# Sageblatt/plate_inverse_problem

Hardware: AMD Instinct MI355X
Metric: freq-solves/sec (forward+adjoint) @20k DOF (higher is better)
Workload: dtype f64; 1 GPU; C3: orthotropic CFRP-like plate, sh_i strip 100x20x2 mm + AP1030, 19353 DOF, 4096 freqs in 40-600 Hz (in total, 4096 on rank 0), forward+adjoint, loss MSE_LOG_AFC + gradient; n_dofs=19353, freqs_total=4096, freqs_rank0=4096, chunk=2048, lanes=2, factorisation=symmetric: A = L U, U = diag(U) L^T implicit, Dirichlet nodes decoupled, nnz_lu=589025

## Files before the change

### include/pfr.h

```cpp
#ifndef PFR_H
#define PFR_H

#include <stddef.h>
#include <stdint.h>

#ifdef __cplusplus
extern "C" {
#endif

#define PFR_API __attribute__((visibility("default")))

#define PFR_OK 0
#define PFR_ERR_ARG 1
#define PFR_ERR_SYMBOLIC 2
#define PFR_ERR_HIP 3
#define PFR_ERR_NOMEM 4
#define PFR_ERR_STATE 5

#define PFR_FLAG_BAD_PIVOT 1
#define PFR_FLAG_BACKWARD_ERROR 2
#define PFR_FLAG_BACKWARD_ERROR_ADJ 4

#define PFR_CHECK_FORWARD 1
#define PFR_CHECK_ADJOINT 2
// ... 76 lines not shown

#define PFR_SCHED_FACTOR_COLS 13
#define PFR_SCHED_PAIR_COLS 9
#define PFR_SCHED_CHAIN_COLS 11
#define PFR_SCHED_SOLVE_COLS 5
#define PFR_SCHED_COLS (PFR_SCHED_FACTOR_COLS + PFR_SCHED_PAIR_COLS + PFR_SCHED_CHAIN_COLS + 3 * PFR_SCHED_SOLVE_COLS)
PFR_API int pfr_symbolic_schedule(const pfr_symbolic* sym, int32_t max_batch, int32_t* dst, int64_t capacity_bytes);
PFR_API int pfr_solver_schedule(const pfr_solver* s, int32_t* dst, int64_t capacity_bytes);

PFR_API int pfr_set_prune(pfr_solver* s, int32_t on);
PFR_API int pfr_symbolic_prune(const pfr_symbolic* sym, int32_t max_batch, const double* rhs, int32_t n_support,
                               const int32_t* index, int32_t* mask, int32_t* sched_active, int32_t* sched_rest,
                               int32_t* sched_full, int64_t capacity_bytes);
PFR_API int32_t pfr_solver_active(const pfr_solver* s, int32_t* mask, int64_t capacity);
PFR_API int pfr_solver_schedule_active(const pfr_solver* s, int32_t* dst, int64_t capacity_bytes);

PFR_API int pfr_solve(pfr_solver* s, int32_t batch, const double* data_dev, int64_t data_stride,
                      const double* b_dev, int64_t b_stride, double* x_dev, int32_t transpose,
                      int32_t* flags_dev, void* stream);

PFR_API int pfr_solve_multi(pfr_solver* s, int32_t batch, int32_t nrhs, const double* data_dev,
                            int64_t data_stride, const double* b_dev, int64_t b_stride, int64_t b_rhs_stride,
                            double* x_dev, int64_t x_rhs_stride, int32_t transpose, int32_t* flags_dev,
                            void* stream);
PFR_API int pfr_matvec(pfr_solver* s, int32_t batch, const double* data_dev, int64_t data_stride,
                       const double* x_dev, int64_t x_stride, double* y_dev, int32_t transpose, void* stream);


PFR_API int pfr_set_stiffness(pfr_solver* s, int32_t n_stiff, const double* stiff_dev ,
                              const double* rhs_weights );
// ... 55 lines not shown
```

### plate_inverse_problem_amd/_native.py

```python
from __future__ import annotations

import ctypes as C
import os
import re

import numpy as np

LIB_PATH = os.environ.get("PFR_LIB") or os.path.join(os.path.dirname(os.path.abspath(__file__)), "_lib", "libpfr.so")
HEADER_PATH = os.path.join(os.path.dirname(os.path.dirname(os.path.abspath(__file__))), "include", "pfr.h")

PFR_OK = 0
PFR_FLAG_BAD_PIVOT = 1
PFR_FLAG_BACKWARD_ERROR = 2
PFR_FLAG_BACKWARD_ERROR_ADJ = 4
PFR_CHECK_FORWARD, PFR_CHECK_ADJOINT, PFR_CHECK_REFINE, PFR_CHECK_CORRECT = 1, 2, 4, 8
PFR_CHECK_REFINE_ADJ = 16
LOSS_NONE, LOSS_MSE, LOSS_RMSE, LOSS_MSE_AFC, LOSS_MSE_LOG_AFC, LOSS_COTANGENT = -1, 0, 1, 2, 3, 4
LOSS_IDS = {"MSE": LOSS_MSE, "RMSE": LOSS_RMSE, "MSE_AFC": LOSS_MSE_AFC, "MSE_LOG_AFC": LOSS_MSE_LOG_AFC}
LOSS_CMSE, LOSS_CRMSE, LOSS_CLOG, LOSS_CCOTANGENT = 16, 17, 18, 19
COMPLEX_LOSS_IDS = {"MSE_COMPLEX": LOSS_CMSE, "RMSE_COMPLEX": LOSS_CRMSE, "MSE_LOG_COMPLEX": LOSS_CLOG}

EXPORT = dict(PERM=0, IPERM=1, FRONTS=2, IDX=3, RELPOS=4, ASM_PTR=5, ASM_COL=6, ASM_NZ=7, EA_PTR=8,
              EA_SRC=9, LEVEL_PTR=10, LEVEL_FRONTS=11, DIRICHLET=12, COUPLING=13)

# ... 39 lines not shown
    "pfr_symbolic_options_default": (None, [C.POINTER(SymbolicOptions)]),
    "pfr_symbolic_create": (C.c_int, [C.c_int32, C.c_int64, _I32P, _I32P, C.POINTER(SymbolicOptions), C.POINTER(_P)]),
    "pfr_symbolic_stats_get": (C.c_int, [_P, C.POINTER(SymbolicStats)]),
    "pfr_symbolic_export": (C.c_int, [_P, C.c_int32, _P, C.c_int64]),
    "pfr_symbolic_destroy": (None, [_P]),
    "pfr_solver_create": (C.c_int, [_P, _I32P, _I32P, C.c_int32, C.c_int32, C.POINTER(_P)]),
    "pfr_solver_destroy": (None, [_P]),
    "pfr_solver_workspace_bytes": (C.c_int64, [_P, C.c_int32]),
    "pfr_solver_max_batch": (C.c_int32, [_P]),
    "pfr_symbolic_schedule": (C.c_int, [_P, C.c_int32, _I32P, C.c_int64]),
    "pfr_solver_schedule": (C.c_int, [_P, _I32P, C.c_int64]),
    "pfr_set_prune": (C.c_int, [_P, C.c_int32]),
    "pfr_symbolic_prune": (C.c_int, [_P, C.c_int32, _DP, C.c_int32, _I32P, _I32P, _I32P, _I32P, _I32P, C.c_int64]),
    "pfr_solver_active": (C.c_int32, [_P, _I32P, C.c_int64]),
    "pfr_solver_schedule_active": (C.c_int, [_P, _I32P, C.c_int64]),
    "pfr_solve": (C.c_int, [_P, C.c_int32, _P, C.c_int64, _P, C.c_int64, _P, C.c_int32, _P, _P]),
    "pfr_matvec": (C.c_int, [_P, C.c_int32, _P, C.c_int64, _P, C.c_int64, _P, C.c_int32, _P]),
    "pfr_set_stiffness": (C.c_int, [_P, C.c_int32, _P, _DP]),
    "pfr_combine": (C.c_int, [_P, _DP, _P, _P]),
    "pfr_set_operator": (C.c_int, [_P, _P, _P]),
    "pfr_set_rhs": (C.c_int, [_P, _DP, C.c_double, C.c_double, C.c_double]),
    "pfr_set_functional": (C.c_int, [_P, C.c_int32, _I32P, _DP, C.c_double]),
    "pfr_sweep": (C.c_int, [_P, C.c_int32, _P, C.c_int32, _P, C.c_double, _P, _P, _P, _P, _P]),
    "pfr_sweep_graph_launches": (C.c_int64, [_P]),
    "pfr_stream_order": (C.c_int, [_P, _P]),
    "pfr_sweep_fresh": (C.c_int, [_P, C.c_int32, _P, C.c_int32, _P, C.c_double, _P, _P, _P, _P, _P]),
    "pfr_jacobian_sweep": (C.c_int, [_P, C.c_int32, _P, _P, _P, _P, _P]),
    "pfr_sweep_complex": (C.c_int, [_P, C.c_int32, _P, _DP, C.c_int32, _P, C.c_double, _P, _P, _P, _P, C.c_int32, _P]),
    "pfr_jacobian_sweep_complex": (C.c_int, [_P, C.c_int32, _P, _DP, _P, _P, _P, _P]),
    "pfr_combine_batch": (C.c_int, [_P, C.c_int32, _DP, _P, _P]),
# ... 162 lines not shown
        st = self.stats()
        r, rp = _f64(rhs)
        sup, sp = _i32(np.asarray(support, dtype=np.int32))
        mask = np.zeros(st["n_fronts"], dtype=np.int32)
        cols = sum(len(c) for _, c in SCHEDULE)
        flat = np.zeros((3, st["n_levels"] * cols), dtype=np.int32)
        check(lib().pfr_symbolic_prune(self._h, int(max_batch), rp, int(sup.size), sp, mask.ctypes.data_as(_I32P),
                                       flat[0].ctypes.data_as(_I32P), flat[1].ctypes.data_as(_I32P),
                                       flat[2].ctypes.data_as(_I32P), flat[0].nbytes),
              "pfr_symbolic_prune")

        def table(row):
            return _schedule(st["n_levels"], lambda dst, cap: C.memmove(dst, row.ctypes.data, row.nbytes))
        return mask, table(flat[0]), table(flat[1]), table(flat[2])

    def __del__(self):
        h = getattr(self, "_h", None)
        if h is not None and _lib is not None:
            _lib.pfr_symbolic_destroy(h)
            self._h = None


class Solver:

    def __init__(self, sym: Symbolic, device_index: int, max_batch: int):
        L = lib()
        self.sym = sym
        self.device_index = int(device_index)
        h = _P()
        _, cp = _i32(sym.colptr)
# ... 10 lines not shown
            _lib.pfr_solver_destroy(h)
            self._h = None

    def schedule(self) -> dict:
        return _schedule(self.sym.stats()["n_levels"], lambda dst, cap: check(
            lib().pfr_solver_schedule(self._h, dst, cap), "pfr_solver_schedule"))

    def set_prune(self, on: bool = True):
        check(lib().pfr_set_prune(self._h, int(bool(on))), "pfr_set_prune")

    def active_fronts(self) -> np.ndarray:
        mask = np.zeros(self.sym.stats()["n_fronts"], dtype=np.int32)
        lib().pfr_solver_active(self._h, mask.ctypes.data_as(_I32P), mask.size)
        return mask

    def schedule_active(self) -> dict:
        return _schedule(self.sym.stats()["n_levels"], lambda dst, cap: check(
            lib().pfr_solver_schedule_active(self._h, dst, cap), "pfr_solver_schedule_active"))

    @staticmethod
    def _stream(t):
        import torch
        return torch.cuda.current_stream(t.device).cuda_stream

    def set_stiffness(self, stiff_nz_k, rhs_weights):
        self._keep["stiff"] = stiff_nz_k
        w, wp = _f64(rhs_weights)
        check(lib().pfr_set_stiffness(self._h, int(stiff_nz_k.shape[1]), _ptr(stiff_nz_k), wp), "pfr_set_stiffness")

    def combine(self, coef: np.ndarray, out):
# ... 121 lines not shown
```

### plate_inverse_problem_amd/csrc/api.cpp

```cpp
#include <hip/hip_runtime.h>

#include <algorithm>
#include <array>
#include <cmath>
#include <cstring>
#include <string>
#include <vector>

#include "launch.hpp"

using pfr::DevPattern;
using pfr::Front;
using pfr::Symbolic;
using pfr::Walk;

struct pfr_symbolic {
  Symbolic S;
};

namespace {
thread_local std::string g_last_error;

int fail(int code, const std::string& msg) {
  g_last_error = msg;
// ... 22 lines not shown
  HIP_TRY(hipMalloc(dst, src.size() * sizeof(T)));
  HIP_TRY(hipMemcpy(*dst, src.data(), src.size() * sizeof(T), hipMemcpyHostToDevice));
  return PFR_OK;
}

int64_t round64(int64_t x) { return (x + 63) / 64 * 64; }

}

struct SolverView {
  std::vector<char> active;
  std::vector<int32_t> level_ptr;
  std::vector<int32_t> tile_ptr, blk_ptr, asm_ptr, item_ptr;
  std::vector<void*> mine;
  int32_t* d_walk = nullptr;
  int post_n = 0;
  int2* post_dir = nullptr;
  int32_t* post_dptr = nullptr;
  int2* post_de = nullptr;
  int32_t* d_level_fronts = nullptr;
  int4* d_tiles = nullptr;
  int4* d_items = nullptr;
  int2* d_orec = nullptr;
  int32_t *d_f0_front = nullptr, *d_f0_ptr = nullptr, *d_f0_nz = nullptr;
  int32_t* d_oxp = nullptr;
  int2* d_ox = nullptr;
  int32_t* d_g1 = nullptr;
  int32_t* d_gxp = nullptr;
  int2* d_gx = nullptr;
  int4* d_blocks = nullptr;
// ... 49 lines not shown
  int2* d_de = nullptr;
  int32_t* d_cslot = nullptr;
  double2* Bc = nullptr;
  std::vector<int32_t> front_of_col, front_parent, front_ns, front_f;
  int fn_dot = 1;
  std::vector<int32_t> front_off, front_col0;
  std::vector<double> a_perm;
  double* d_aP = nullptr;
  int32_t* d_noslot = nullptr;
  double2* WVk = nullptr;
  double2* YVk = nullptr;
  double2* fn_parts = nullptr;
  double2* fcoef = nullptr;
  int contract_walk = 1;
  double2* kpart = nullptr;
  double2 *F = nullptr, *WV = nullptr, *X = nullptr, *Y = nullptr, *XA = nullptr, *G = nullptr, *Y2 = nullptr;
  double2* XR = nullptr;
  int32_t *d_rptr = nullptr, *d_ridx = nullptr, *d_rnz = nullptr;
  int32_t *d_cptr = nullptr, *d_cidx = nullptr, *d_cnz = nullptr;
  double2 *DX = nullptr, *DL = nullptr, *Kdir = nullptr;
  int4* d_uent = nullptr;
  int n_uent = 0;
  double* d_se = nullptr;
  int n_kdir = 0;
  double2 *partial = nullptr, *tq = nullptr;
  double *freqs = nullptr, *loss_terms = nullptr;
  double* fr0 = nullptr;
  double2* h0 = nullptr;
  double2 *mscale = nullptr, *cpart = nullptr;
  int scale_corr = 1;
// ... 373 lines not shown
int set_reach(pfr_solver* s, SolverView& v, int which, const std::vector<int32_t>& prows) {
  std::vector<int32_t> mark, list;
  pfr::reach_lists(s->front_of_col, s->front_parent, v.level_ptr, v.level_fronts_host, prows, mark, list,
                   v.reach_ptr[which]);
  v.reach_host[which].assign(mark.begin(), mark.end());
  v.fn_ready = false;
  if (&v == s && s->act) s->act->fn_ready = false;
  pfr::schedule_reach(v.sched, v.reach_ptr, &v != s ? &s->reach_ptr : nullptr);
  HIP_TRY(hipMemcpy(v.d_reach[which], mark.data(), mark.size() * 4, hipMemcpyHostToDevice));
  if (!list.empty()) HIP_TRY(hipMemcpy(v.d_reach_fronts[which], list.data(), list.size() * 4, hipMemcpyHostToDevice));
  return PFR_OK;
}

void run_walk(pfr_solver* s, const SolverView& v, const pfr::ChunkOp& op, const Walk& w, int nvalid, hipStream_t st) {
  const bool fwd = w.sys == Walk::FORWARD;
  const pfr::ResidArgs d{.ptr = fwd ? s->d_rptr : s->d_cptr, .idx = fwd ? s->d_ridx : s->d_cidx,
                         .nzs = fwd ? s->d_rnz : s->d_cnz, .n = s->n, .K = op.K, .M = op.M, .freqs = op.freqs,
                         .data = w.data, .data_stride = w.ds, .nvalid = nvalid, .rhsP = w.rd.rhsP,
                         .beta_re = w.rd.beta_re, .beta_im = w.rd.beta_im, .mass_sum = w.rd.mass_sum, .B = w.rd.B,
                         .b_stride = w.rd.b_stride, .perm = s->P.perm, .G = w.rd.G, .walk = v.d_walk,
                         .se = w.contract ? s->stiff : nullptr, .kpart = w.contract ? s->kpart : nullptr,
                         .glist = w.glist};
  const int n_stiff = w.contract ? s->n_stiff : 0;
  pfr::launch_residual(w.mat, w.rhs, d, n_stiff, s->res_unroll, op.pop, w.X, s->Fc, w.R, w.check ? s->d_berr_acc : nullptr,
                       st, w.Mu, w.Mu ? s->cpart : nullptr);
  if (!w.check) return;
  pfr::launch_berr_finish(s->d_berr_acc, s->Fc, nvalid, s->check_tol,
                          fwd ? PFR_FLAG_BACKWARD_ERROR : PFR_FLAG_BACKWARD_ERROR_ADJ, s->flags,
                          w.q0 >= 0 ? s->berr_out : nullptr, w.q0, w.sys, st);
}

void contract_rows(pfr_solver* s, const double2* lam, const double2* x, int nv, hipStream_t st) {
  pfr::launch_contract_eg(s->d_uent, s->n_uent, s->d_se, s->n_stiff, lam, x, s->Fc, nv, s->partial, st);
}

int upload_view(pfr_solver* s, SolverView& v, const Symbolic& S, const pfr::Plan& pl, const pfr::Knobs& knobs) {
  int rc;
  const size_t own0 = s->owned.size();
  const int nf = (int)S.fronts.size();
  v.active = pl.active;
// ... 29 lines not shown
  if (&v != s) v.mine.assign(s->owned.begin() + own0, s->owned.end());
  return PFR_OK;
}

void release_view(pfr_solver* s, SolverView*& v) {
  if (!v) return;
  (void)hipDeviceSynchronize();
  for (void* p : v->mine) {
    s->owned.erase(std::remove(s->owned.begin(), s->owned.end(), p), s->owned.end());
    (void)hipFree(p);
  }
  delete v;
  v = nullptr;
}

int make_view(pfr_solver* s, const std::vector<char>& mask, bool keep0, SolverView** out) {
  pfr::Plan pl;
  std::string perr;
  if (pfr::build_plan(s->S, s->sched.knobs.blk_min, pl, perr, &mask)) return fail(PFR_ERR_ARG, perr);
  auto* v = new SolverView();
  int rc = upload_view(s, *v, s->S, pl, s->sched.knobs);
  std::vector<pfr::I2> dir, de;
  std::vector<int32_t> dptr(1, 0);
  for (size_t d = 0; d < s->h_dir.size() && rc == PFR_OK; ++d) {
    if (!mask[s->front_of_col[s->h_dir[d].x]]) continue;
    dir.push_back(s->h_dir[d]);
    de.insert(de.end(), s->h_de.begin() + s->h_dptr[d], s->h_de.begin() + s->h_dptr[d + 1]);
    dptr.push_back((int32_t)de.size());
  }
  const size_t own0 = s->owned.size();
// ... 30 lines not shown
  for (size_t t = 0; t < mask.size(); ++t) {
    if (mask[t]) continue;
    const int32_t a = s->front_col0[t], b = a + s->front_ns[t];
    s->unl_rows.emplace_back(a, b);
  }
  std::sort(s->unl_rows.begin(), s->unl_rows.end());
  size_t k = 0;
  for (size_t i = 1; i < s->unl_rows.size(); ++i) {
    if (s->unl_rows[i].first == s->unl_rows[k].second)
      s->unl_rows[k].second = s->unl_rows[i].second;
    else
      s->unl_rows[++k] = s->unl_rows[i];
  }
  if (!s->unl_rows.empty()) s->unl_rows.resize(k + 1);
  s->unl_dirty = true;
  return make_view(s, mask, true, &s->act);
}

}

extern "C" {

const char* pfr_version(void) { return "pfr 0.1.0 (gfx950, frequency-minor multifrontal)"; }
const char* pfr_last_error(void) { return g_last_error.c_str(); }

void pfr_symbolic_options_default(pfr_symbolic_options* o) {
  pfr::SymbolicOptions d;
  o->leaf_size = d.leaf_size;
  o->ordering = d.ordering;
  o->relax_small = d.relax_small;
  o->relax_mid = d.relax_mid;
// ... 115 lines not shown
  HIP_TRY(hipSetDevice(device));
  const Symbolic& S = sym->S;
  auto* s = new pfr_solver();
  auto bail = [&](int rc) {
    delete s;
    return rc;
  };
  s->device = device;
  auto knob = [](const char* name, int def, int lo, int hi) {
    const char* e = getenv(name);
    return e ? std::max(lo, std::min(hi, atoi(e))) : def;
  };
  s->res_unroll = knob("PFR_RES_UNROLL", 8, 4, 8) == 8 ? 8 : 4;
  s->fn_dot = knob("PFR_FN_DOT", 1, 0, 1);
  s->contract_walk = knob("PFR_CONTRACT_WALK", 1, 0, 1);
  s->scale_corr = knob("PFR_SCALE_CORR", 1, 0, 1);
  s->graph_mode = knob("PFR_GRAPH", 0, 0, 1);
  s->n = S.n;
  s->nnz = S.nnz;
  s->Fc = round64(max_batch);
  s->level_ptr = S.level_ptr;
  s->perm = S.perm;
  s->iperm = S.iperm;
  const pfr::Knobs knobs = pfr::knobs_from_env(s->Fc);
  pfr::Plan pl;
  std::string perr;
  if (pfr::build_plan(S, knobs.blk_min, pl, perr)) return bail(fail(PFR_ERR_ARG, perr));
  s->sym = pl.sym;
  Front* d_fronts = nullptr;
  int rc = PFR_OK;
// ... 174 lines not shown
  const int64_t nf = (int64_t)s->front_ns.size();
  int32_t count = 0;
  for (int64_t t = 0; t < nf; ++t) {
    const int32_t a = s->act ? s->act->active[t] != 0 : 1;
    count += a;
    if (mask && t < cap) mask[t] = a;
  }
  return s->act ? count : (int32_t)nf;
}

int pfr_solver_schedule_active(const pfr_solver* s, int32_t* dst, int64_t cap) {
  if (!s) return fail(PFR_ERR_ARG, "null solver");
  return schedule_out(s->act ? s->act->sched : s->sched, dst, cap);
}

int pfr_set_timing(pfr_solver* s, int32_t enable) {
  if (!s) return fail(PFR_ERR_ARG, "null solver");
  ++s->gen;
  s->timing = enable == 0 ? 0 : (enable | 1);
  return PFR_OK;
}

namespace {
int complete_adjoint(pfr_solver* s) {
  if (!s->act || !s->last_pruned || !s->last_adj || s->comp_done) return PFR_OK;
  int rc;
  if (!s->comp) {
    std::vector<char> mask(s->act->active);
    for (char& m : mask) m = !m;
    if ((rc = make_view(s, mask, false, &s->comp))) return rc;
// ... 138 lines not shown
  s->n_stiff = n_stiff;
  std::memset(&s->e, 0, sizeof(s->e));
  for (int k = 0; k < n_stiff; ++k) s->e.re[k] = w[k];
  HIP_TRY(hipSetDevice(s->device));
  if (!s->partial) {
    const int64_t parts = std::max<int64_t>(pfr::contract_eg_parts(s->n_uent), s->Fc / 64);
    int rc = s->alloc(&s->partial, parts * 18);
    if (rc) return rc;
  }
  if (!s->d_se) {
    int rc = s->alloc(&s->d_se, (int64_t)18 * (s->n_uent + 4));
    if (rc) return rc;
  }
  pfr::launch_gather_entries(s->d_uent, s->n_uent + 4, stiff_dev, n_stiff, s->d_se, nullptr);
  HIP_TRY(hipStreamSynchronize(nullptr));
  return PFR_OK;
}

int pfr_combine(pfr_solver* s, const double* coef, double* K_out, void* stream) {
  if (!s || !coef || !K_out) return fail(PFR_ERR_ARG, "null argument");
  if (!s->stiff) return fail(PFR_ERR_STATE, "pfr_set_stiffness not called");
  HIP_TRY(hipSetDevice(s->device));
  pfr::CoefPack c{};
  for (int k = 0; k < s->n_stiff; ++k) {
    c.re[k] = coef[2 * k];
    c.im[k] = coef[2 * k + 1];
  }
  pfr::launch_combine(s->stiff, s->n_stiff, s->nnz, c, reinterpret_cast<double2*>(K_out), (hipStream_t)stream);
  LAUNCH_TRY();
  return PFR_OK;
// ... 716 lines not shown
```

### plate_inverse_problem_amd/csrc/asan_driver.cpp

```cpp
#include <algorithm>
#include <cstdio>
#include <cstdlib>
#include <string>
#include <vector>

#include "plan.hpp"
#include "symbolic.hpp"

namespace {
template <class T>
bool rd(FILE* f, T* p, size_t n) {
  return fread(p, sizeof(T), n, f) == n;
}

struct Views {
  pfr::Plan P[2];
  std::vector<char> mask[2];
  std::vector<int32_t> full_ptr[2], ptr[2][2];
};
std::string build_views(const pfr::Symbolic& S, int bm, int32_t load_row, const std::vector<int32_t>& sup,
                        const std::vector<int32_t>& foc, const std::vector<int32_t>& par, Views& V) {
  std::vector<double> rhs(S.n, 0.0);
  rhs[load_row] = 1.0;
  V.mask[0] = pfr::loaded_fronts(S, rhs.data());
// ... 2 lines not shown
  if (!V.mask[0][foc[load_row]]) return "the loaded row's front is not loaded";
  std::vector<int32_t> rows[2] = {{load_row}, sup}, mark, list;
  for (size_t c = 0; c < S.cpl_p.size(); ++c) rows[0].push_back(S.cpl_p[c]);
  for (int w = 0; w < 2; ++w) pfr::reach_lists(foc, par, S.level_ptr, S.level_fronts, rows[w], mark, list, V.full_ptr[w]);
  std::string err;
  for (int side = 0; side < 2; ++side) {
    if (pfr::build_plan(S, bm, V.P[side], err, &V.mask[side])) return err;
    for (int w = side; w < 2; ++w)
      pfr::reach_lists(foc, par, V.P[side].level_ptr, V.P[side].level_fronts, pfr::rows_in(S, V.mask[side], rows[w]), mark,
                       list, V.ptr[side][w]);
  }
  for (size_t l = 0; l + 1 < S.level_ptr.size(); ++l)
    if (V.P[0].level_ptr[l + 1] - V.P[0].level_ptr[l] + V.P[1].level_ptr[l + 1] - V.P[1].level_ptr[l] !=
        S.level_ptr[l + 1] - S.level_ptr[l])
      return "views do not partition a level";
  return "";
}
std::string check_views(const pfr::Symbolic& S, const Views& V, int64_t Fc, const pfr::Knobs& k) {
  for (int side = 0; side < 2; ++side) {
    std::string e = pfr::check_plan(S, V.P[side], Fc);
    if (e.empty()) e = pfr::check_schedule(S, V.P[side], pfr::level_schedule(S, V.P[side], Fc, k, V.ptr[side], &V.full_ptr));
    if (!e.empty()) return std::string(side == 0 ? "loaded view: " : "unloaded view: ") + e;
  }
  return "";
}

std::string fused_forest(bool big) {
  const std::vector<int> ms[2] = {{1, 2, 3, 4, 4}, big ? std::vector<int>{3, 6, 9} : std::vector<int>{2, 2, 4}};
  const int s[2] = {10, big ? 12 : 6};
  std::vector<std::vector<int32_t>> col;
// ... 232 lines not shown
```

### plate_inverse_problem_amd/csrc/device_types.hpp

```cpp
#pragma once

#include <hip/hip_runtime.h>

#include <cstdint>

#include "../../include/pfr.h"
#include "plan.hpp"
#include "symbolic.hpp"

namespace pfr {

struct DevPattern {
  const Front* fronts;
  const int32_t* idx;
  const int32_t* relpos;
  const int32_t* row_front;
  const int32_t* asm_ptr;
  const int32_t* asm_col;
  const int32_t* asm_nz;
  const int32_t* ea_ptr;
  const int32_t* ea_src;
  const int32_t* perm;
  const int32_t* prow;
  const int32_t* pcol;
// ... 49 lines not shown
  const double2* K = nullptr;
  const double* M = nullptr;
  const double* freqs = nullptr;
  const double2* data = nullptr;
  int64_t data_stride = 0;
  int nvalid = 1;
  const double* rhsP = nullptr;
  double beta_re = 0, beta_im = 0, mass_sum = 0;
  const double2* B = nullptr;
  int64_t b_stride = 0;
  const int* perm = nullptr;
  const double2* G = nullptr;
  const int* walk = nullptr;
  const double* se = nullptr;
  double2* kpart = nullptr;
  const int* glist = nullptr;
};

constexpr int LOSS_UNIT = PFR_LOSS_COTANGENT + 1;

struct FunctionalArgs {
  int32_t cpx;
  double axis[3];
  double2* h_out;
  double2* h0;
  int32_t n_support;
  const int32_t* pidx;
  const double* a;
  double ts;
  int32_t loss_type;
// ... 7 lines not shown
```

### plate_inverse_problem_amd/csrc/kernels.hip

```cpp
#include <hip/hip_runtime.h>

#include <cstdint>
#include <cstdlib>

#include <algorithm>
#include <atomic>
#include <type_traits>

#include "launch.hpp"

namespace pfr {

using cplx = double2;

__device__ __forceinline__ cplx cadd(cplx a, cplx b) { return make_double2(a.x + b.x, a.y + b.y); }
__device__ __forceinline__ cplx cmul(cplx a, cplx b) {
  return make_double2(fma(a.x, b.x, -a.y * b.y), fma(a.x, b.y, a.y * b.x));
}
__device__ __forceinline__ cplx cfms(cplx c, cplx a, cplx b) {
  return make_double2(fma(-a.x, b.x, fma(a.y, b.y, c.x)), fma(-a.x, b.y, fma(-a.y, b.x, c.y)));
}
__device__ __forceinline__ cplx cscale(cplx a, double m) { return make_double2(a.x * m, a.y * m); }
__device__ __forceinline__ cplx crecip(cplx b) {
  double d = fma(b.x, b.x, b.y * b.y);
// ... 2307 lines not shown
  dd_sub_prod(rh.x, rl.x, -a.y, x.y);
  dd_sub_prod(rh.y, rl.y, a.x, x.y);
  dd_sub_prod(rh.y, rl.y, a.y, x.x);
}

template <int MODE>
__device__ __forceinline__ cplx resid_entry(const ResidArgs& A, const cplx* __restrict__ dq, int nz, double om2) {
  if (MODE == 0) {
    const cplx k = A.K[nz];
    return make_double2(fma(-om2, A.M[nz], k.x), k.y);
  }
  return dq[nz];
}

constexpr int RES_WPE = 4;
template <int MODE, int RHS, bool DOT = false, int NSK = 0, bool CMP = DOT, int RU = 4, bool POP = false>
__global__ __launch_bounds__(256) __attribute__((amdgpu_waves_per_eu(NSK > 0 ? RES_WPE : 1))) void k_residual(ResidArgs A, const cplx* __restrict__ X, int64_t Fc,
                                                  cplx* __restrict__ R, double* __restrict__ acc,
                                                  const cplx* __restrict__ Mu, cplx* __restrict__ cpart, PopArgs pop) {
  const int64_t lid = xcd_swizzle(blockIdx.x + (int64_t)gridDim.x * blockIdx.y, (int64_t)gridDim.x * gridDim.y);
  const int bx = (int)(lid % gridDim.x), by = A.glist ? A.glist[lid / gridDim.x] : (int)(lid / gridDim.x);
  if (by < 0) return;
  const int64_t q = (int64_t)by * 64 + (threadIdx.x & 63);
  const int wave0 = __builtin_amdgcn_readfirstlane(bx * (blockDim.x >> 6) + (threadIdx.x >> 6));
  const int nwaves = gridDim.x * (blockDim.x >> 6);
  if (POP) {
    const int m = pop_member(pop, q);
    A.K += m * pop.nnz;
    if (RHS == 0) {
      const cplx beta = pop.beta[m];
      A.beta_re = beta.x;
      A.beta_im = beta.y;
// ... 88 lines not shown
  }
  if (DOT) {
    __shared__ cplx sdot[4][64];
    const int w = threadIdx.x >> 6, lane = threadIdx.x & 63;
    sdot[w][lane] = dot;
    __syncthreads();
    if (w == 0) {
      cplx t = sdot[0][lane];
      for (int k = 1; k < (int)(blockDim.x >> 6); ++k) t = cadd(t, sdot[k][lane]);
      cpart[(int64_t)bx * Fc + q] = t;
    }
  }
  if (NSK > 0) {
    __shared__ cplx sks[4][64];
    const int w = threadIdx.x >> 6, lane = threadIdx.x & 63;
#pragma unroll
    for (int k = 0; k < NSK; ++k) {
      __syncthreads();
      sks[w][lane] = ks[k];
      __syncthreads();
      if (w == 0)
        A.kpart[((int64_t)bx * NSK + k) * Fc + q] =
            cadd(cadd(sks[0][lane], sks[1][lane]), cadd(sks[2][lane], sks[3][lane]));
    }
  }
  if (!acc) return;
  if (bad) berr = __longlong_as_double(0x7ff0000000000000LL);
  atomicMax(reinterpret_cast<unsigned long long*>(acc + q), (unsigned long long)__double_as_longlong(berr));
}

__device__ __forceinline__ void loss_term(int loss_type, double fr, cplx r, double& term, double& dl) {
  const double rabs = sqrt(r.x * r.x + r.y * r.y);
  term = 0.0;
  dl = 0.0;
  switch (loss_type) {
    case PFR_LOSS_MSE: {
      const double dre = fr - r.x;
      term = dre * dre + r.y * r.y;
      dl = 2.0 * dre;
// ... 416 lines not shown
  for (int t = blockIdx.x * 4 + (threadIdx.x >> 6); t < nrows; t += gridDim.x * 4) {
    const int64_t o = (int64_t)rows[t] * Fc + q;
    Y0[o] = cadd(cadd(cmul(c0, Y0[o]), cmul(c1, Y1[o])), cmul(c2, Y2[o]));
  }
}

__global__ void k_gather_entries(const int4* __restrict__ ent, int nent, const double* __restrict__ stiff, int ns,
                                 double* __restrict__ se) {
  const int e = blockIdx.x * blockDim.x + threadIdx.x;
  if (e >= nent) return;
  const int4 en = ent[e];
  const bool ij = en.x >= 0 && en.y >= 0;
  for (int k = 0; k < ns; ++k) se[(int64_t)e * ns + k] = ij ? stiff[(int64_t)en.y * ns + k] : 0.0;
}

template <int NS, int EW, bool MS>
__global__ __launch_bounds__(256) void k_contract_eg(const int4* __restrict__ ent, int nent,
                                                     const double* __restrict__ se, const cplx* __restrict__ Lam,
                                                     const cplx* __restrict__ X, int64_t Fc, int nvalid,
                                                     const cplx* __restrict__ msc, cplx* __restrict__ partial) {
  const int lane = threadIdx.x & 63;
  const int wv = __builtin_amdgcn_readfirstlane(blockIdx.x * (blockDim.x >> 6) + (threadIdx.x >> 6));
  const int e0 = min(wv * EW, nent - 1);
  int64_t oi[EW], oj[EW];
#pragma unroll
  for (int u = 0; u < EW; ++u) {
    const int4 en = ent[min(e0 + u, nent - 1)];
    oi[u] = (int64_t)max(en.w, 0) * Fc + lane;
    oj[u] = (int64_t)max(en.x, 0) * Fc + lane;
  }
// ... 471 lines not shown
}

void launch_tangent_spmv(const int* ptr, const int* idx, const int* nzs, int nrows, const double2* Kd,
                         const double2* X, int64_t Fc, const double* rhsP, double2 beta, double2* Y, int accumulate,
                         hipStream_t st) {
  LAUNCH(k_tangent_spmv, dim3((nrows + 3) / 4, (unsigned)(Fc / 64)), dim3(256), st, ptr, idx, nzs, nrows, Kd, X, Fc,
         rhsP, beta, Y, accumulate);
}


void launch_residual(Mat mode, Rhs rhs, const ResidArgs& a, int n_stiff, int unroll, const PopArgs& pop, const double2* X,
                     int64_t Fc, double2* R, double* acc, hipStream_t st, const double2* Mu, double2* cpart) {
  if (pop.member && mode != 0) return;
  const int rh = mode == 0 ? (rhs == 0 ? 0 : 2) : (rhs == 1 ? 1 : 2);
  const bool dot = mode == 0 && rhs == 0 && Mu;
  const int nsk = dot && a.kpart && (n_stiff == 12 || n_stiff == 18) ? n_stiff : 0;
  const bool cmp = dot || R;
  const int ru = mode == 0 && rh == 2 && !cmp && unroll == 8 ? 8 : 4;
  dispatch([&](auto md, auto rhc, auto dt, auto nk, auto cm, auto un, auto pp) {
    constexpr int MD = CV(md), RH = CV(rhc), NK = CV(nk), RU = CV(un);
    constexpr bool DT = CV(dt), CM = CV(cm), PP = CV(pp);
    if constexpr ((RH == 2 || RH == MD) && (!DT || (MD == 0 && RH == 0 && CM)) && (NK == 0 || DT) &&
                  (RU == 4 || (MD == 0 && RH == 2 && !CM)) && (!PP || MD == 0))
      LAUNCH((k_residual<MD, RH, DT, NK, CM, RU, PP>), dim3((unsigned)residual_parts(a.n), (unsigned)(a.glist ? REFINE_CAP : Fc / 64)),
             dim3(256), st, a, X, Fc, R, acc, Mu, cpart, pop);
  }, pick<0, 1>(mode), pick<0, 1, 2>(rh), flag(dot), pick<0, 12, 18>(nsk), flag(cmp), pick<4, 8>(ru),
     flag(pop.member != nullptr));
}

void launch_correct_finish(const FunctionalArgs& A, const double* fr0, const double2* cpart, int nparts, int64_t Fc,
                           int nvalid, int64_t q0, double* fr_out, double* loss_terms, double2* mscale,
                           const ChunkOp& op, hipStream_t st, double* gind, double2* tq) {
  RhsScale bsc;
  bsc.freqs = op.freqs;
  bsc.mass_sum = op.mass_sum;
  bsc.beta_re = op.beta_re;
  bsc.beta_im = op.beta_im;
  dispatch([&](auto pp, auto cx) {
    if constexpr (!(CV(pp) && CV(cx)))
      LAUNCH((k_correct_finish<CV(pp), CV(cx)>), dim3((unsigned)(Fc / 64)), dim3(256), st, A, fr0, cpart, nparts, Fc,
             nvalid, q0, fr_out, loss_terms, mscale, gind, tq, bsc, op.pop);
// ... 24 lines not shown
                               int64_t q0, double2* G, hipStream_t st) {
  LAUNCH(k_functional_tangent, dim3((unsigned)((Fc + 63) / 64)), dim3(64), st, A, X, DX, Fc, nvalid, q0, G);
}

void launch_functional(const FunctionalArgs& A, const double2* X, int64_t Fc, int nvalid, int64_t q0, double* fr_out,
                       double* loss_terms, double2* G, hipStream_t st) {
  with_bool(A.cpx != 0, [&](auto cx) {
    LAUNCH(k_functional<CV(cx)>, dim3((unsigned)((Fc + 63) / 64)), dim3(64), st, A, X, Fc, nvalid, q0, fr_out, loss_terms,
           G);
  });
}

void launch_gather_entries(const int4* ent, int nent, const double* stiff, int ns, double* se, hipStream_t st) {
  if (nent <= 0) return;
  LAUNCH(k_gather_entries, dim3((nent + 255) / 256), dim3(256), st, ent, nent, stiff, ns, se);
}


void launch_contract_eg(const int4* ent, int nent, const double* se, int n_stiff, const double2* Lam, const double2* X,
                        int64_t Fc, int nvalid, double2* partial, hipStream_t st, const double2* msc) {
  dispatch([&](auto ns, auto ms) {
    LAUNCH((k_contract_eg<CV(ns), CEG_EW, CV(ms)>), dim3(contract_eg_parts(nent)), dim3(256), st, ent, nent, se, Lam, X, Fc,
           nvalid, msc, partial);
  }, pick<12, 18>(n_stiff), flag(msc != nullptr));
}

void launch_rhs_dot(const int* sup, const double* val, int n_sup, const double2* Lam, int64_t Fc, double2* t_out,
                    hipStream_t st, const double2* msc) {
  LAUNCH(k_rhs_dot, dim3((unsigned)((Fc + 63) / 64)), dim3(64), st, sup, val, n_sup, Lam, Fc, msc, t_out);
}
// ... 112 lines not shown
```

### plate_inverse_problem_amd/csrc/launch.hpp

```cpp
#pragma once

#include "device_types.hpp"

namespace pfr {

struct ChunkOp {
  const double2* K = nullptr;
  const double* M = nullptr;
  const double* freqs = nullptr;
  const double* rhsP = nullptr;
  double beta_re = 0, beta_im = 0, mass_sum = 0;
  PopArgs pop;
};

enum Tri { TRI_L = 0, TRI_U = 1, TRI_UT = 2, TRI_LT = 3 };
enum Rhs { RHS_OPERATOR = 0, RHS_BATCH = 1, RHS_VECTOR = 2, RHS_OPERATOR_DIR = 3 };
enum Reach { REACH_ALL = -1, REACH_RHS = 0, REACH_SUPPORT = 1 };
enum Mat { MAT_OPERATOR = 0, MAT_BATCH = 1 };

const char* launch_refused();

void launch_combine(const double* stiff, int n_stiff, int64_t nnz, const CoefPack& coef, double2* K, hipStream_t st);
void launch_combine_batch(const double* stiff, int n_stiff, int64_t nnz, const double2* coef, int n_members,
                          double2* K, hipStream_t st);
// ... 24 lines not shown
                          double* fr_out, double* loss_terms, double2* G, double2* fcoef, hipStream_t st);
void launch_fn_combine(const int* rows, int nrows, const double2* fcoef, double2* const* Yk, int64_t Fc, hipStream_t st);
void launch_usolve2(const DevPattern& P, const int* lvl, const PairLevel& r, int ngroups, const double2* F, int64_t Fc,
                    const double2* Y0, double2* X0, const int* reach0, const int* skip0, const double2* Y1, double2* X1,
                    const int* reach1, hipStream_t st);
void launch_tangent_spmv(const int* ptr, const int* idx, const int* nzs, int nrows, const double2* Kd,
                         const double2* X, int64_t Fc, const double* rhsP, double2 beta, double2* Y, int accumulate,
                         hipStream_t st);
void launch_functional_tangent(const FunctionalArgs& A, const double2* X, const double2* DX, int64_t Fc, int nvalid,
                               int64_t q0, double2* G, hipStream_t st);
void launch_functional(const FunctionalArgs& A, const double2* X, int64_t Fc, int nvalid, int64_t q0, double* fr_out,
                       double* loss_terms, double2* G, hipStream_t st);
void launch_contract_eg(const int4* ent, int nent, const double* se, int n_stiff, const double2* Lam, const double2* X,
                        int64_t Fc, int nvalid, double2* partial, hipStream_t st, const double2* msc = nullptr);
void launch_gather_entries(const int4* ent, int nent, const double* stiff, int ns, double* se, hipStream_t st);
void launch_rhs_dot(const int* sup, const double* val, int n_sup, const double2* Lam, int64_t Fc, double2* t_out,
                    hipStream_t st, const double2* msc = nullptr);
void launch_reduce(const double2* partial, int nparts, int n_stiff, const double2* t_q, const CoefPack& e,
                   const double* loss_terms, int nvalid, int64_t Fc, double2* w_out, double* loss_out,
                   hipStream_t st);
void launch_contract_q(const int4* ent, int nent, const double* se, int n_stiff, const double2* Lam, const double2* X,
                       int n, int64_t Fc, double2* kpart, hipStream_t st);
void launch_jac_finish(const double2* kpart, int nparts, int n_stiff, const double2* msc, const double2* t_q,
                       const CoefPack& e, int nvalid, int64_t Fc, double2* jc, hipStream_t st);
void launch_dirichlet_rhs(Rhs src, const DirArgs& d, const PopArgs& pop, int n_crow, const RhsArgs& rd, double2* G,
                          double2* Bc, int64_t Fc, hipStream_t st);
void launch_dirichlet_post(const DirArgs& d, const PopArgs& pop, int n_dir, double2* X, int64_t Fc, hipStream_t st,
                           const int* glist = nullptr);
void launch_residual(Mat mode, Rhs rhs, const ResidArgs& a, int n_stiff, int unroll, const PopArgs& pop, const double2* X,
                     int64_t Fc, double2* R, double* acc, hipStream_t st, const double2* Mu = nullptr,
// ... 50 lines not shown
```

### plate_inverse_problem_amd/csrc/plan.cpp

```cpp
#include "plan.hpp"

#include <algorithm>
#include <climits>
#include <cstdio>
#include <cstdlib>
#include <utility>

namespace pfr {

Workspace workspace(const Symbolic& S, int64_t Fc, int n_crow) {
  Workspace w;
  const int64_t n = S.n;
  w.F = S.factor_entries * Fc;
  w.WV = S.total_rows * Fc;
  w.nvec = n * Fc;
  w.n_nvec = 7;
  w.cpart = (int64_t)residual_parts(S.n) * Fc;
  w.kpart = (int64_t)residual_parts(S.n) * 18 * Fc;
  w.berr_acc = 2 * Fc;
  w.gind = Fc / 64;
  w.Bc = (int64_t)std::max(1, n_crow) * Fc;
  if (S.symmetric) {
    w.WVk = 3 * S.total_rows * Fc;
    w.YVk = 2 * n * Fc;
// ... 386 lines not shown
  }
  std::vector<char> loaded_root(nfr, 0);
  auto load = [&](int32_t p) {
    if (p >= 0 && p < S.n && front_of_col[p] >= 0) loaded_root[root[front_of_col[p]]] = 1;
  };
  for (int32_t p = 0; p < S.n; ++p)
    if (rhs_perm[p] != 0.0) load(p);
  for (size_t c = 0; c < S.cpl_p.size(); ++c)
    if (rhs_perm[S.dir_p[S.cpl_dir[c]]] != 0.0) load(S.cpl_p[c]);
  const std::vector<char> by_value(loaded_root);
  for (size_t c = 0; c < S.cpl_p.size(); ++c)
    if (by_value[root[front_of_col[S.cpl_p[c]]]]) load(S.dir_p[S.cpl_dir[c]]);
  std::vector<char> mask(nfr);
  for (int t = 0; t < nfr; ++t) mask[t] = loaded_root[root[t]];
  return mask;
}

std::vector<int32_t> rows_in(const Symbolic& S, const std::vector<char>& mask, const std::vector<int32_t>& prows) {
  std::vector<char> row_on(S.n, 0);
  for (size_t t = 0; t < S.fronts.size(); ++t)
    if (mask[t])
      for (int a = 0; a < S.fronts[t].ns; ++a) row_on[S.fronts[t].col0 + a] = 1;
  std::vector<int32_t> out;
  for (int32_t p : prows)
    if (p >= 0 && p < S.n && row_on[p]) out.push_back(p);
  return out;
}

void reach_lists(const std::vector<int32_t>& front_of_col, const std::vector<int32_t>& front_parent,
                 const std::vector<int32_t>& level_ptr, const std::vector<int32_t>& level_fronts,
// ... 402 lines not shown
```

### plate_inverse_problem_amd/csrc/plan.hpp

```cpp
#pragma once

#include <algorithm>
#include <array>
#include <cstdint>
#include <string>
#include <vector>

#include "symbolic.hpp"

namespace pfr {

struct I2 {
  int32_t x, y;
};
struct I4 {
  int32_t x, y, z, w;
};

constexpr int SCHUR_SR = 1, SCHUR_SC = 1, SCHUR_QG = 64 / (SCHUR_SR * SCHUR_SC);
constexpr int SCHUR_TM = 4, SCHUR_TN = 4;
static_assert(SCHUR_SR * SCHUR_SC * SCHUR_QG == 64, "one wavefront per super-tile");
constexpr int SCHUR_TILE = SCHUR_TM * SCHUR_TN * SCHUR_SR * SCHUR_SC;
constexpr int SCHUR_BLK = 16;
constexpr int SCHUR_BLK_IDS = 16 * SCHUR_BLK;
// ... 71 lines not shown
  int n_uent = 0;
};

struct Workspace {
  int64_t F = 0, WV = 0, nvec = 0;
  int64_t n_nvec = 0;
  int64_t cpart = 0, kpart = 0, partial = 0, berr_acc = 0, gind = 0;
  int64_t WVk = 0, YVk = 0, fn_parts = 0, fcoef = 0, Bc = 0;
  int64_t bytes = 0;
};
Workspace workspace(const Symbolic& S, int64_t Fc, int n_crow);

int build_plan(const Symbolic& S, int blk_min, Plan& P, std::string& err, const std::vector<char>* mask = nullptr);

std::vector<char> loaded_fronts(const Symbolic& S, const double* rhs_perm);
std::vector<int32_t> rows_in(const Symbolic& S, const std::vector<char>& mask, const std::vector<int32_t>& prows);

void reach_lists(const std::vector<int32_t>& front_of_col, const std::vector<int32_t>& front_parent,
                 const std::vector<int32_t>& level_ptr, const std::vector<int32_t>& level_fronts,
                 const std::vector<int32_t>& prows, std::vector<int32_t>& mark, std::vector<int32_t>& list,
                 std::vector<int32_t>& ptr);

std::string check_plan(const Symbolic& S, const Plan& P, int64_t Fc);

struct Knobs {
  int solve_wmax = 8;
  int fac_wmax = 16;
  int fac_g_wg = 0;
  int fac_gbig = 4;
  int fac_g_ns = 64;
// ... 68 lines not shown
```

Baseline: 108,900 freq-solves/s.

## Contract only stiffness matrices live on visited rows in residual kernel

```diff
diff --git a/include/pfr.h b/include/pfr.h
--- a/include/pfr.h
+++ b/include/pfr.h
@@ -114,6 +114,9 @@
                                int32_t* sched_full, int64_t capacity_bytes);
 PFR_API int32_t pfr_solver_active(const pfr_solver* s, int32_t* mask, int64_t capacity);
 PFR_API int pfr_solver_schedule_active(const pfr_solver* s, int32_t* dst, int64_t capacity_bytes);
+PFR_API int32_t pfr_symbolic_live(const pfr_symbolic* sym, const double* rhs, int32_t prune, int32_t n_stiff,
+                                  const double* stiff_host, uint32_t* live);
+PFR_API int32_t pfr_solver_live(const pfr_solver* s, uint32_t* live, int32_t* compact);
 
 PFR_API int pfr_solve(pfr_solver* s, int32_t batch, const double* data_dev, int64_t data_stride,
                       const double* b_dev, int64_t b_stride, double* x_dev, int32_t transpose,
diff --git a/plate_inverse_problem_amd/_native.py b/plate_inverse_problem_amd/_native.py
--- a/plate_inverse_problem_amd/_native.py
+++ b/plate_inverse_problem_amd/_native.py
@@ -77,6 +77,8 @@
     "pfr_symbolic_prune": (C.c_int, [_P, C.c_int32, _DP, C.c_int32, _I32P, _I32P, _I32P, _I32P, _I32P, C.c_int64]),
     "pfr_solver_active": (C.c_int32, [_P, _I32P, C.c_int64]),
     "pfr_solver_schedule_active": (C.c_int, [_P, _I32P, C.c_int64]),
+    "pfr_symbolic_live": (C.c_int32, [_P, _DP, C.c_int32, C.c_int32, _DP, C.POINTER(C.c_uint32)]),
+    "pfr_solver_live": (C.c_int32, [_P, C.POINTER(C.c_uint32), _I32P]),
     "pfr_solve": (C.c_int, [_P, C.c_int32, _P, C.c_int64, _P, C.c_int64, _P, C.c_int32, _P, _P]),
     "pfr_matvec": (C.c_int, [_P, C.c_int32, _P, C.c_int64, _P, C.c_int64, _P, C.c_int32, _P]),
     "pfr_set_stiffness": (C.c_int, [_P, C.c_int32, _P, _DP]),
@@ -269,6 +271,15 @@
             return _schedule(st["n_levels"], lambda dst, cap: C.memmove(dst, row.ctypes.data, row.nbytes))
         return mask, table(flat[0]), table(flat[1]), table(flat[2])
 
+    def live(self, rhs, stiff_nz_k, prune: bool = True) -> list:
+        r, rp = _f64(rhs)
+        s, sp = _f64(stiff_nz_k)
+        bits = C.c_uint32(0)
+        n = lib().pfr_symbolic_live(self._h, rp, int(bool(prune)), int(s.shape[1]), sp, C.byref(bits))
+        if n < 0:
+            raise NativeError("pfr_symbolic_live: bad arguments (needs a symmetric analysis)")
+        return [k for k in range(int(s.shape[1])) if (bits.value >> k) & 1]
+
     def __del__(self):
         h = getattr(self, "_h", None)
         if h is not None and _lib is not None:
@@ -309,6 +320,11 @@
         lib().pfr_solver_active(self._h, mask.ctypes.data_as(_I32P), mask.size)
         return mask
 
+    def live(self) -> tuple:
+        bits, compact = C.c_uint32(0), C.c_int32(0)
+        lib().pfr_solver_live(self._h, C.byref(bits), C.byref(compact))
+        return [k for k in range(18) if (bits.value >> k) & 1], bool(compact.value)
+
     def schedule_active(self) -> dict:
         return _schedule(self.sym.stats()["n_levels"], lambda dst, cap: check(
             lib().pfr_solver_schedule_active(self._h, dst, cap), "pfr_solver_schedule_active"))
diff --git a/plate_inverse_problem_amd/csrc/api.cpp b/plate_inverse_problem_amd/csrc/api.cpp
--- a/plate_inverse_problem_amd/csrc/api.cpp
+++ b/plate_inverse_problem_amd/csrc/api.cpp
@@ -60,6 +60,9 @@
   std::vector<int32_t> tile_ptr, blk_ptr, asm_ptr, item_ptr;
   std::vector<void*> mine;
   int32_t* d_walk = nullptr;
+  uint32_t live = 0;
+  int n_live = 0;
+  double* d_se_live = nullptr;
   int post_n = 0;
   int2* post_dir = nullptr;
   int32_t* post_dptr = nullptr;
@@ -139,6 +142,9 @@
   double2* fcoef = nullptr;
   int contract_walk = 1;
   double2* kpart = nullptr;
+  int contract_live = 1, live_unroll = 8;
+  std::vector<uint32_t> stiff_bits;
+  int32_t* d_live_bad = nullptr;
   double2 *F = nullptr, *WV = nullptr, *X = nullptr, *Y = nullptr, *XA = nullptr, *G = nullptr, *Y2 = nullptr;
   double2* XR = nullptr;
   int32_t *d_rptr = nullptr, *d_ridx = nullptr, *d_rnz = nullptr;
@@ -542,16 +548,19 @@
 
 void run_walk(pfr_solver* s, const SolverView& v, const pfr::ChunkOp& op, const Walk& w, int nvalid, hipStream_t st) {
   const bool fwd = w.sys == Walk::FORWARD;
+  const bool compact = w.contract && v.d_se_live;
+  const unsigned all = w.contract ? (1u << s->n_stiff) - 1u : 0u;
   const pfr::ResidArgs d{.ptr = fwd ? s->d_rptr : s->d_cptr, .idx = fwd ? s->d_ridx : s->d_cidx,
                          .nzs = fwd ? s->d_rnz : s->d_cnz, .n = s->n, .K = op.K, .M = op.M, .freqs = op.freqs,
                          .data = w.data, .data_stride = w.ds, .nvalid = nvalid, .rhsP = w.rd.rhsP,
                          .beta_re = w.rd.beta_re, .beta_im = w.rd.beta_im, .mass_sum = w.rd.mass_sum, .B = w.rd.B,
                          .b_stride = w.rd.b_stride, .perm = s->P.perm, .G = w.rd.G, .walk = v.d_walk,
-                         .se = w.contract ? s->stiff : nullptr, .kpart = w.contract ? s->kpart : nullptr,
-                         .glist = w.glist};
+                         .se = compact ? v.d_se_live : w.contract ? s->stiff : nullptr,
+                         .kpart = w.contract ? s->kpart : nullptr, .live = compact ? v.live : all,
+                         .nslot = w.contract ? s->n_stiff : 0, .glist = w.glist};
   const int n_stiff = w.contract ? s->n_stiff : 0;
-  pfr::launch_residual(w.mat, w.rhs, d, n_stiff, s->res_unroll, op.pop, w.X, s->Fc, w.R, w.check ? s->d_berr_acc : nullptr,
-                       st, w.Mu, w.Mu ? s->cpart : nullptr);
+  pfr::launch_residual(w.mat, w.rhs, d, n_stiff, w.contract ? s->live_unroll : s->res_unroll, op.pop, w.X, s->Fc, w.R,
+                       w.check ? s->d_berr_acc : nullptr, st, w.Mu, w.Mu ? s->cpart : nullptr);
   if (!w.check) return;
   pfr::launch_berr_finish(s->d_berr_acc, s->Fc, nvalid, s->check_tol,
                           fwd ? PFR_FLAG_BACKWARD_ERROR : PFR_FLAG_BACKWARD_ERROR_ADJ, s->flags,
@@ -611,6 +620,34 @@
   v = nullptr;
 }
 
+int update_live(pfr_solver* s, SolverView& v) {
+  if (v.d_se_live) {
+    (void)hipDeviceSynchronize();
+    s->owned.erase(std::remove(s->owned.begin(), s->owned.end(), (void*)v.d_se_live), s->owned.end());
+    v.mine.erase(std::remove(v.mine.begin(), v.mine.end(), (void*)v.d_se_live), v.mine.end());
+    (void)hipFree(v.d_se_live);
+    v.d_se_live = nullptr;
+  }
+  v.live = s->n_stiff ? (1u << s->n_stiff) - 1u : 0u;
+  v.n_live = s->n_stiff;
+  if (!s->stiff || !s->sym || s->stiff_bits.empty()) return PFR_OK;
+  v.live = pfr::live_stiffness(s->S, &v == s ? nullptr : &v.active, s->stiff_bits);
+  v.n_live = __builtin_popcount(v.live);
+  if (!s->contract_live || v.n_live >= s->n_stiff || (v.n_live != 6 && v.n_live != 12)) return PFR_OK;
+  int rc;
+  if (!s->d_live_bad && (rc = s->alloc(&s->d_live_bad, 1))) return rc;
+  if ((rc = s->alloc(&v.d_se_live, s->nnz * v.n_live))) return rc;
+  if (&v != s) v.mine.push_back(v.d_se_live);
+  HIP_TRY(hipMemsetAsync(s->d_live_bad, 0, 4, nullptr));
+  HIP_TRY(hipMemsetAsync(v.d_se_live, 0, (size_t)s->nnz * v.n_live * 8, nullptr));
+  pfr::launch_gather_live(v.d_walk, s->n, s->d_rptr, s->d_rnz, s->stiff, s->n_stiff, v.live, v.n_live, v.d_se_live,
+                          s->d_live_bad, nullptr);
+  int32_t bad = 0;
+  HIP_TRY(hipMemcpy(&bad, s->d_live_bad, 4, hipMemcpyDeviceToHost));
+  if (bad) return fail(PFR_ERR_STATE, "a stiffness matrix outside the live list is non-zero on a visited entry");
+  return PFR_OK;
+}
+
 int make_view(pfr_solver* s, const std::vector<char>& mask, bool keep0, SolverView** out) {
   pfr::Plan pl;
   std::string perr;
@@ -671,7 +708,8 @@
   }
   if (!s->unl_rows.empty()) s->unl_rows.resize(k + 1);
   s->unl_dirty = true;
-  return make_view(s, mask, true, &s->act);
+  if (int rc = make_view(s, mask, true, &s->act)) return rc;
+  return update_live(s, *s->act);
 }
 
 }
@@ -817,6 +855,8 @@
   s->res_unroll = knob("PFR_RES_UNROLL", 8, 4, 8) == 8 ? 8 : 4;
   s->fn_dot = knob("PFR_FN_DOT", 1, 0, 1);
   s->contract_walk = knob("PFR_CONTRACT_WALK", 1, 0, 1);
+  s->contract_live = knob("PFR_CONTRACT_LIVE", 1, 0, 1);
+  s->live_unroll = knob("PFR_LIVE_UNROLL", 8, 4, 8) == 8 ? 8 : 4;
   s->scale_corr = knob("PFR_SCALE_CORR", 1, 0, 1);
   s->graph_mode = knob("PFR_GRAPH", 0, 0, 1);
   s->n = S.n;
@@ -1021,6 +1061,29 @@
   return schedule_out(s->act ? s->act->sched : s->sched, dst, cap);
 }
 
+int32_t pfr_symbolic_live(const pfr_symbolic* sym, const double* rhs, int32_t prune, int32_t n_stiff,
+                          const double* stiff_host, uint32_t* live) {
+  if (!sym || !rhs || !stiff_host || n_stiff <= 0 || n_stiff > 18 || !sym->S.symmetric) return -1;
+  const Symbolic& S = sym->S;
+  std::vector<char> mask;
+  if (prune) {
+    std::vector<double> rp(S.n);
+    for (int p = 0; p < S.n; ++p) rp[p] = rhs[S.perm[p]];
+    mask = pfr::loaded_fronts(S, rp.data());
+  }
+  const uint32_t l = pfr::live_stiffness(S, prune ? &mask : nullptr, pfr::stiffness_bits(stiff_host, S.nnz, n_stiff));
+  if (live) *live = l;
+  return __builtin_popcount(l);
+}
+
+int32_t pfr_solver_live(const pfr_solver* s, uint32_t* live, int32_t* compact) {
+  if (!s) return -1;
+  const SolverView& v = sweeps_pruned(s) ? *s->act : static_cast<const SolverView&>(*s);
+  if (live) *live = v.live;
+  if (compact) *compact = v.d_se_live != nullptr;
+  return v.n_live;
+}
+
 int pfr_set_timing(pfr_solver* s, int32_t enable) {
   if (!s) return fail(PFR_ERR_ARG, "null solver");
   ++s->gen;
@@ -1189,6 +1252,15 @@
   }
   pfr::launch_gather_entries(s->d_uent, s->n_uent + 4, stiff_dev, n_stiff, s->d_se, nullptr);
   HIP_TRY(hipStreamSynchronize(nullptr));
+  s->stiff_bits.clear();
+  if (s->sym) {
+    std::vector<double> host((size_t)s->nnz * n_stiff);
+    HIP_TRY(hipMemcpy(host.data(), stiff_dev, host.size() * 8, hipMemcpyDeviceToHost));
+    s->stiff_bits = pfr::stiffness_bits(host.data(), s->nnz, n_stiff);
+  }
+  if (int rc = update_live(s, *s)) return rc;
+  if (s->act)
+    if (int rc = update_live(s, *s->act)) return rc;
   return PFR_OK;
 }
 
diff --git a/plate_inverse_problem_amd/csrc/asan_driver.cpp b/plate_inverse_problem_amd/csrc/asan_driver.cpp
--- a/plate_inverse_problem_amd/csrc/asan_driver.cpp
+++ b/plate_inverse_problem_amd/csrc/asan_driver.cpp
@@ -40,6 +40,17 @@
     if (V.P[0].level_ptr[l + 1] - V.P[0].level_ptr[l] + V.P[1].level_ptr[l + 1] - V.P[1].level_ptr[l] !=
         S.level_ptr[l + 1] - S.level_ptr[l])
       return "views do not partition a level";
+  std::vector<double> stiff(3 * S.nnz, 0.0);
+  bool any[2] = {false, false};
+  for (int64_t e = 0; e < S.nnz; ++e) {
+    const int side = V.mask[0][foc[S.prow[e]]] ? 0 : 1;
+    stiff[3 * e + side] = 1.0 + e;
+    any[side] = true;
+  }
+  const std::vector<uint32_t> bits = pfr::stiffness_bits(stiff.data(), S.nnz, 3);
+  for (int side = 0; side < 2; ++side)
+    if (pfr::live_stiffness(S, &V.mask[side], bits) != (any[side] ? 1u << side : 0u)) return "live stiffness list of a view";
+  if (pfr::live_stiffness(S, nullptr, bits) != ((any[0] ? 1u : 0u) | (any[1] ? 2u : 0u))) return "live stiffness list";
   return "";
 }
 std::string check_views(const pfr::Symbolic& S, const Views& V, int64_t Fc, const pfr::Knobs& k) {
diff --git a/plate_inverse_problem_amd/csrc/device_types.hpp b/plate_inverse_problem_amd/csrc/device_types.hpp
--- a/plate_inverse_problem_amd/csrc/device_types.hpp
+++ b/plate_inverse_problem_amd/csrc/device_types.hpp
@@ -87,6 +87,8 @@
   const int* walk = nullptr;
   const double* se = nullptr;
   double2* kpart = nullptr;
+  unsigned live = 0;
+  int nslot = 0;
   const int* glist = nullptr;
 };
 
diff --git a/plate_inverse_problem_amd/csrc/kernels.hip b/plate_inverse_problem_amd/csrc/kernels.hip
--- a/plate_inverse_problem_amd/csrc/kernels.hip
+++ b/plate_inverse_problem_amd/csrc/kernels.hip
@@ -2345,8 +2345,11 @@
 }
 
 constexpr int RES_WPE = 4;
+#ifndef RES_WPE_LIVE
+#define RES_WPE_LIVE 4
+#endif
 template <int MODE, int RHS, bool DOT = false, int NSK = 0, bool CMP = DOT, int RU = 4, bool POP = false>
-__global__ __launch_bounds__(256) __attribute__((amdgpu_waves_per_eu(NSK > 0 ? RES_WPE : 1))) void k_residual(ResidArgs A, const cplx* __restrict__ X, int64_t Fc,
+__global__ __launch_bounds__(256) __attribute__((amdgpu_waves_per_eu(NSK > 0 ? (NSK <= 6 ? RES_WPE_LIVE : RES_WPE) : 1))) void k_residual(ResidArgs A, const cplx* __restrict__ X, int64_t Fc,
                                                   cplx* __restrict__ R, double* __restrict__ acc,
                                                   const cplx* __restrict__ Mu, cplx* __restrict__ cpart, PopArgs pop) {
   const int64_t lid = xcd_swizzle(blockIdx.x + (int64_t)gridDim.x * blockIdx.y, (int64_t)gridDim.x * gridDim.y);
@@ -2465,15 +2468,21 @@
   if (NSK > 0) {
     __shared__ cplx sks[4][64];
     const int w = threadIdx.x >> 6, lane = threadIdx.x & 63;
+    unsigned left = A.live;
 #pragma unroll
     for (int k = 0; k < NSK; ++k) {
+      const int slot = __builtin_ctz(left);
+      left &= left - 1;
       __syncthreads();
       sks[w][lane] = ks[k];
       __syncthreads();
       if (w == 0)
-        A.kpart[((int64_t)bx * NSK + k) * Fc + q] =
+        A.kpart[((int64_t)bx * A.nslot + slot) * Fc + q] =
             cadd(cadd(sks[0][lane], sks[1][lane]), cadd(sks[2][lane], sks[3][lane]));
     }
+    if (w == 0)
+      for (unsigned dead = ~A.live & ((1u << A.nslot) - 1u); dead; dead &= dead - 1)
+        A.kpart[((int64_t)bx * A.nslot + __builtin_ctz(dead)) * Fc + q] = make_double2(0.0, 0.0);
   }
   if (!acc) return;
   if (bad) berr = __longlong_as_double(0x7ff0000000000000LL);
@@ -2920,6 +2929,28 @@
   for (int k = 0; k < ns; ++k) se[(int64_t)e * ns + k] = ij ? stiff[(int64_t)en.y * ns + k] : 0.0;
 }
 
+__global__ void k_gather_live(const int* __restrict__ walk, int n, const int* __restrict__ ptr,
+                              const int* __restrict__ nzs, const double* __restrict__ stiff, int ns, unsigned live,
+                              int nl, double* __restrict__ se_live, int* __restrict__ bad) {
+  const int t = blockIdx.x * blockDim.x + threadIdx.x;
+  if (t >= n) return;
+  const int p = walk[t];
+  if (p < 0) return;
+  for (int e = ptr[p]; e < ptr[p + 1]; ++e) {
+    const int64_t nz = nzs[e];
+    int i = 0;
+    for (int k = 0; k < ns; ++k) {
+      const double v = stiff[nz * ns + k];
+      if ((live >> k) & 1u) {
+        if (i < nl) se_live[nz * nl + i] = v;
+        ++i;
+      } else if (v != 0.0) {
+        *bad = 1;
+      }
+    }
+  }
+}
+
 template <int NS, int EW, bool MS>
 __global__ __launch_bounds__(256) void k_contract_eg(const int4* __restrict__ ent, int nent,
                                                      const double* __restrict__ se, const cplx* __restrict__ Lam,
@@ -3421,17 +3452,21 @@
   if (pop.member && mode != 0) return;
   const int rh = mode == 0 ? (rhs == 0 ? 0 : 2) : (rhs == 1 ? 1 : 2);
   const bool dot = mode == 0 && rhs == 0 && Mu;
-  const int nsk = dot && a.kpart && (n_stiff == 12 || n_stiff == 18) ? n_stiff : 0;
+  const int nsk = dot && a.kpart && (n_stiff == 12 || n_stiff == 18) ? __builtin_popcount(a.live) : 0;
+  if (nsk && ((nsk != 6 && nsk != 12 && nsk != 18) || nsk > n_stiff || a.nslot != n_stiff || (a.live >> n_stiff))) {
+    dyn_ok(false, "k_residual: live stiffness list");
+    return;
+  }
   const bool cmp = dot || R;
-  const int ru = mode == 0 && rh == 2 && !cmp && unroll == 8 ? 8 : 4;
+  const int ru = unroll == 8 && ((mode == 0 && rh == 2 && !cmp) || nsk == 6) ? 8 : 4;
   dispatch([&](auto md, auto rhc, auto dt, auto nk, auto cm, auto un, auto pp) {
     constexpr int MD = CV(md), RH = CV(rhc), NK = CV(nk), RU = CV(un);
     constexpr bool DT = CV(dt), CM = CV(cm), PP = CV(pp);
     if constexpr ((RH == 2 || RH == MD) && (!DT || (MD == 0 && RH == 0 && CM)) && (NK == 0 || DT) &&
-                  (RU == 4 || (MD == 0 && RH == 2 && !CM)) && (!PP || MD == 0))
+                  (RU == 4 || (MD == 0 && RH == 2 && !CM) || NK == 6) && (!PP || MD == 0))
       LAUNCH((k_residual<MD, RH, DT, NK, CM, RU, PP>), dim3((unsigned)residual_parts(a.n), (unsigned)(a.glist ? REFINE_CAP : Fc / 64)),
              dim3(256), st, a, X, Fc, R, acc, Mu, cpart, pop);
-  }, pick<0, 1>(mode), pick<0, 1, 2>(rh), flag(dot), pick<0, 12, 18>(nsk), flag(cmp), pick<4, 8>(ru),
+  }, pick<0, 1>(mode), pick<0, 1, 2>(rh), flag(dot), pick<0, 6, 12, 18>(nsk), flag(cmp), pick<4, 8>(ru),
      flag(pop.member != nullptr));
 }
 
@@ -3486,6 +3521,12 @@
 void launch_gather_entries(const int4* ent, int nent, const double* stiff, int ns, double* se, hipStream_t st) {
   if (nent <= 0) return;
   LAUNCH(k_gather_entries, dim3((nent + 255) / 256), dim3(256), st, ent, nent, stiff, ns, se);
+}
+
+void launch_gather_live(const int* walk, int n, const int* ptr, const int* nzs, const double* stiff, int ns,
+                        unsigned live, int nl, double* se_live, int* bad, hipStream_t st) {
+  if (n <= 0) return;
+  LAUNCH(k_gather_live, dim3((n + 255) / 256), dim3(256), st, walk, n, ptr, nzs, stiff, ns, live, nl, se_live, bad);
 }
 
 
diff --git a/plate_inverse_problem_amd/csrc/launch.hpp b/plate_inverse_problem_amd/csrc/launch.hpp
--- a/plate_inverse_problem_amd/csrc/launch.hpp
+++ b/plate_inverse_problem_amd/csrc/launch.hpp
@@ -62,6 +62,8 @@
 void launch_contract_eg(const int4* ent, int nent, const double* se, int n_stiff, const double2* Lam, const double2* X,
                         int64_t Fc, int nvalid, double2* partial, hipStream_t st, const double2* msc = nullptr);
 void launch_gather_entries(const int4* ent, int nent, const double* stiff, int ns, double* se, hipStream_t st);
+void launch_gather_live(const int* walk, int n, const int* ptr, const int* nzs, const double* stiff, int ns,
+                        unsigned live, int nl, double* se_live, int* bad, hipStream_t st);
 void launch_rhs_dot(const int* sup, const double* val, int n_sup, const double2* Lam, int64_t Fc, double2* t_out,
                     hipStream_t st, const double2* msc = nullptr);
 void launch_reduce(const double2* partial, int nparts, int n_stiff, const double2* t_q, const CoefPack& e,
diff --git a/plate_inverse_problem_amd/csrc/plan.cpp b/plate_inverse_problem_amd/csrc/plan.cpp
--- a/plate_inverse_problem_amd/csrc/plan.cpp
+++ b/plate_inverse_problem_amd/csrc/plan.cpp
@@ -424,6 +424,26 @@
   std::vector<char> mask(nfr);
   for (int t = 0; t < nfr; ++t) mask[t] = loaded_root[root[t]];
   return mask;
+}
+
+std::vector<uint32_t> stiffness_bits(const double* stiff, int64_t nnz, int n_stiff) {
+  std::vector<uint32_t> bits(nnz, 0);
+  for (int64_t nz = 0; nz < nnz; ++nz)
+    for (int k = 0; k < n_stiff; ++k)
+      if (stiff[nz * n_stiff + k] != 0.0) bits[nz] |= 1u << k;
+  return bits;
+}
+
+uint32_t live_stiffness(const Symbolic& S, const std::vector<char>* mask, const std::vector<uint32_t>& bits) {
+  std::vector<char> row_on(S.n, mask ? 0 : 1);
+  if (mask)
+    for (size_t t = 0; t < S.fronts.size(); ++t)
+      if ((*mask)[t])
+        for (int a = 0; a < S.fronts[t].ns; ++a) row_on[S.fronts[t].col0 + a] = 1;
+  uint32_t live = 0;
+  for (int64_t nz = 0; nz < S.nnz && nz < (int64_t)bits.size(); ++nz)
+    if (row_on[S.prow[nz]]) live |= bits[nz];
+  return live;
 }
 
 std::vector<int32_t> rows_in(const Symbolic& S, const std::vector<char>& mask, const std::vector<int32_t>& prows) {
diff --git a/plate_inverse_problem_amd/csrc/plan.hpp b/plate_inverse_problem_amd/csrc/plan.hpp
--- a/plate_inverse_problem_amd/csrc/plan.hpp
+++ b/plate_inverse_problem_amd/csrc/plan.hpp
@@ -109,6 +109,8 @@
 int build_plan(const Symbolic& S, int blk_min, Plan& P, std::string& err, const std::vector<char>* mask = nullptr);
 
 std::vector<char> loaded_fronts(const Symbolic& S, const double* rhs_perm);
+std::vector<uint32_t> stiffness_bits(const double* stiff, int64_t nnz, int n_stiff);
+uint32_t live_stiffness(const Symbolic& S, const std::vector<char>* mask, const std::vector<uint32_t>& bits);
 std::vector<int32_t> rows_in(const Symbolic& S, const std::vector<char>& mask, const std::vector<int32_t>& prows);
 
 void reach_lists(const std::vector<int32_t>& front_of_col, const std::vector<int32_t>& front_parent,
```

Result: faster. 111,100 freq-solves/s, median of 6 (+2.0%).
